# KiloHertzian/Open-Headstage

Hardware: AMD Instinct MI355X
Metric: Msamples/s stereo 48 kHz (4×512-tap HRIR conv + 10-band EQ); % HBM3E peak (higher is better)
Workload: dtype f32

## Files before the change

### open_headstage_amd/csrc/eq_quad_ring_body.hpp

```cpp
#pragma once
#include "kernels.h"
#include "eq_ring64_body.hpp"
#include "eq_quad_ring_asm.inc"
#include "eq_quad_ring_cl_asm.inc"
#include <type_traits>

namespace ohs {

constexpr int kQuadGroup = 16;
constexpr int kQuadK = EQ_QUAD_RING_K;
constexpr int kQp0003 = 0xC0, kQp0033 = 0xF0, kQp0012 = 0x90, kQp0101 = 0x44;

struct QuadRegs { float Z0, Z1, Zp, G, P; };
enum { kQuadLoopCluster, kQuadLoopLone, kQuadLoopFill };

template <int CTRL>
__device__ __forceinline__ float quad_dpp(float src)
{
    return __int_as_float(__builtin_amdgcn_update_dpp(0, __float_as_int(src), CTRL, 0xf, 0xf, true));
}

template <int LOOP = kQuadLoopCluster>
__device__ __forceinline__ void eq_quad_ring_wave(const float *in, float *out, long long stream_stride, long long ch_stride,
                                                  long long n, int n_chains, int nb, const EqPassTable &tab,
                                                  float *__restrict__ state, long long chain)
{
    constexpr int G = kQuadGroup, K = kQuadK;
    static_assert(K == 8, "the operand list below names x0 .. x7");
    static_assert(EQ_QUAD_RING_CL_HOLD == 1, "the clobber list below names one holding register, v20");
    if (chain >= n_chains) return;
    const int lane = threadIdx.x & 63, q = lane >> 2, role = lane & 3;
    const int n32 = (int)n;
    const bool band = q < nb, conv = q >= 12;
    const int j = band ? q : 0;
    const float C1 = role < 2 ? 1.0f : !band ? 0.0f : role == 2 ? tab.a2[j] : tab.a1[j];
    const float C2 = !band ? (role < 2 ? 0.0f : 1.0f) : role == 0 ? tab.b2[j] : role == 1 ? tab.b1[j] : role == 2 ? tab.b0[j] : 1.0f;
    const long long base = (chain >> 1) * stream_stride + (chain & 1) * ch_stride;
    const float *src0 = in + base;
    float *dst0 = out + base;
    float *state0 = state + chain * (kEqStateSlots * 2);
    const bool st_band = band && role >= 2;
    const unsigned state_off = (unsigned)(tab.slot[j] * 2 + (role == 2 ? 1 : 0)) * 4u;
    const float s_init = st_band ? ring2_ld(state0, state_off) : 0.0f;
    float s_save = s_init;
    const int t_in = 4 * q + 2;
    const int xs = (role == 0 ? 71 : role == 1 ? 69 : role == 2 ? 62 : 60) - 4 * q;
    const int ss = (role == 0 ? -1 : -3) - 4 * q;
    const bool st_lane = conv && (role == 0 || role == 3), inj_lane = conv && role >= 2;
    auto load_x = [&](int g) -> float {
        const int i = g * G + xs;
        return (conv && (unsigned)i < (unsigned)n32) ? ring2_ld(src0, (unsigned)i * 4u) : 0.0f;
    };
    QuadRegs r = {0.0f, 0.0f, 0.0f, 0.0f, 0.0f};
    float xcur = load_x(-1), xnext = load_x(0);

    const int g_hi = (n32 + 1) / G;
    const int iters = g_hi - 5 >= K ? (g_hi - 5) / K : 0;
    const int g1 = iters ? g_hi : -1, g0 = iters ? g_hi - iters * K : -1;
    float x2 = 0.0f, x3 = 0.0f, x4 = 0.0f, x5 = 0.0f, x6 = 0.0f, x7 = 0.0f;
    if (iters) {
        x2 = load_x(g0 + 2); x3 = load_x(g0 + 3); x4 = load_x(g0 + 4);
        x5 = load_x(g0 + 5); x6 = load_x(g0 + 6); x7 = load_x(g0 + 7);
    }

    enum { kPlain, kStore, kInjectB, kInjectA };
    auto group_cpp = [&](int g, auto with_state) {
        constexpr bool STATE = decltype(with_state)::value;
        const float xnext2 = load_x(g + 2);
        auto step = [&](auto kind, float &zc, const float zo, int s) {
            const int stp = g * G + s;
            zc = quad_dpp<kWaveRor1>(r.Zp) + r.G;
            r.Zp = quad_dpp<kQp0003>(zo) * C2;
            if constexpr (kind() == kStore) {
                const int yi = stp + ss;
                if (st_lane && (unsigned)yi < (unsigned)n32) ring2_st(dst0, (unsigned)yi * 4u, zc);
            } else if constexpr (kind() == kInjectB) {
                const float xb = quad_dpp<kQp0101>(xcur);
                r.Zp = inj_lane ? xb : r.Zp;
            } else if constexpr (kind() == kInjectA) {
                r.Zp = inj_lane ? xnext : r.Zp;
            }
            r.P = quad_dpp<kQp0033>(zc) * C1;
            r.G = quad_dpp<kQp0012>(zc) - r.P;
            if constexpr (STATE) {
                r.G = (st_band && stp == t_in) ? s_init : r.G;
                s_save = (st_band && stp == n32 + t_in) ? r.G : s_save;
            }
        };
        using Plain = std::integral_constant<int, kPlain>;
        auto plain_pairs = [&](int s0, int s1) {
#pragma unroll 1
            for (int s = s0; s < s1; s += 2) {
                step(Plain{}, r.Z1, r.Z0, s);
                step(Plain{}, r.Z0, r.Z1, s + 1);
            }
        };
        plain_pairs(1, 6);
        step(Plain{}, r.Z1, r.Z0, 7);
        step(std::integral_constant<int, kStore>{}, r.Z0, r.Z1, 8);
        step(std::integral_constant<int, kInjectB>{}, r.Z1, r.Z0, 9);
        step(Plain{}, r.Z0, r.Z1, 10);
        plain_pairs(11, 14);
        step(std::integral_constant<int, kStore>{}, r.Z1, r.Z0, 15);
        step(std::integral_constant<int, kInjectA>{}, r.Z0, r.Z1, 16);
        xcur = xnext;
        xnext = xnext2;
    };

    const int g_total = (n32 + 62 + G - 1) / G;
    int g = -1;
    const int head_end = iters ? g0 : g_total;
#pragma unroll 1
    for (; g < head_end && (g < 3 || !iters); ++g) group_cpp(g, std::true_type{});
#pragma unroll 1
    for (; g < head_end; ++g) group_cpp(g, std::false_type{});
    if (iters) {
        const unsigned bytes = (unsigned)n32 * 4u;
        const ring64_rsrc_t rin = ring64_rsrc(src0, bytes), rout = ring64_rsrc(dst0, bytes);
        unsigned voff_st = st_lane ? (unsigned)(G * (g0 - 1) + 8 + ss) * 4u : 0xFFFFF000u;
        unsigned voff_ld = conv ? (unsigned)(G * g0 + xs) * 4u : 0xFFFFF000u;
        const unsigned inc_ld = conv ? 4u * G * K : 0u, inc_st = st_lane ? 4u * G * K : 0u;
        unsigned cnt = 0u - (unsigned)__builtin_amdgcn_readfirstlane(iters);
#ifdef OHS_EXPERIMENTS
        if constexpr (LOOP == kQuadLoopFill) {
            unsigned fill = 0u;
            asm volatile(
                "s_nop 4\n"
                EQ_QUAD_RING_LOOP_FILL
                : [Z0] "+{v2}"(r.Z0), [Z1] "+{v3}"(r.Z1), [Zp] "+{v4}"(r.Zp), [Gr] "+{v5}"(r.G), [P] "+{v6}"(r.P),
                  [vs] "+{v0}"(voff_st), [vl] "+{v1}"(voff_ld), [x0] "+{v11}"(xcur), [x1] "+{v12}"(xnext), [x2] "+{v13}"(x2),
                  [x3] "+{v14}"(x3), [x4] "+{v15}"(x4), [x5] "+{v16}"(x5), [x6] "+{v17}"(x6), [x7] "+{v18}"(x7),
                  [F] "+{v19}"(fill), [cnt] "+s"(cnt)
                : [C1] "{v7}"(C1), [C2] "{v8}"(C2), [incl] "{v9}"(inc_ld), [incs] "{v10}"(inc_st), [rin] "s"(rin), [rout] "s"(rout)
                : "memory", "scc", "vcc");
        } else if constexpr (LOOP == kQuadLoopLone) {
            asm volatile(
                "s_nop 4\n"
                EQ_QUAD_RING_LOOP
                : [Z0] "+{v2}"(r.Z0), [Z1] "+{v3}"(r.Z1), [Zp] "+{v4}"(r.Zp), [Gr] "+{v5}"(r.G), [P] "+{v6}"(r.P),
                  [vs] "+{v0}"(voff_st), [vl] "+{v1}"(voff_ld), [x0] "+{v11}"(xcur), [x1] "+{v12}"(xnext), [x2] "+{v13}"(x2),
                  [x3] "+{v14}"(x3), [x4] "+{v15}"(x4), [x5] "+{v16}"(x5), [x6] "+{v17}"(x6), [x7] "+{v18}"(x7), [cnt] "+s"(cnt)
                : [C1] "{v7}"(C1), [C2] "{v8}"(C2), [incl] "{v9}"(inc_ld), [incs] "{v10}"(inc_st), [rin] "s"(rin), [rout] "s"(rout)
                : "memory", "scc", "vcc");
        } else
#endif
        asm volatile(
            "s_nop 4\n"
            EQ_QUAD_RING_CL_LOOP
            : [Z0] "+{v2}"(r.Z0), [Z1] "+{v3}"(r.Z1), [Zp] "+{v4}"(r.Zp), [Gr] "+{v5}"(r.G), [P] "+{v6}"(r.P),
              [vs] "+{v0}"(voff_st), [vl] "+{v1}"(voff_ld), [x0] "+{v11}"(xcur), [x1] "+{v12}"(xnext), [x2] "+{v13}"(x2),
              [x3] "+{v14}"(x3), [x4] "+{v15}"(x4), [x5] "+{v16}"(x5), [x6] "+{v17}"(x6), [x7] "+{v18}"(x7), [cnt] "+s"(cnt)
            : [C1] "{v7}"(C1), [C2] "{v8}"(C2), [incl] "{v9}"(inc_ld), [incs] "{v10}"(inc_st), [rin] "s"(rin), [rout] "s"(rout)
            : "memory", "scc", "vcc", "v20");
        g = g1;
#pragma unroll 1
        for (; g < g_total; ++g) group_cpp(g, std::true_type{});
    }
    if (st_band) ring2_st(state0, state_off, s_save);
}

}
```

Baseline: 27340.

## Rewrite quad-ring head/tail with buffer ops and 8-deep rotating prefetch

Restructures the C++ head and tail of the quad-ring EQ kernel. Loads and stores now go through raw buffer intrinsics with an out-of-range sentinel offset instead of branches. The head loop is unrolled into an 8-register rotating prefetch that mirrors the asm steady-state loop. Stores are deferred to a per-group port step, and the state injection and extraction are split so each part only runs where it is needed. The aim is to remove divergent branches and load latency stalls in the prologue and epilogue. The cost is more code, dummy stores at the start, and some risk in the index alignment logic.

```diff
diff --git a/open_headstage_amd/csrc/eq_quad_ring_body.hpp b/open_headstage_amd/csrc/eq_quad_ring_body.hpp
--- a/open_headstage_amd/csrc/eq_quad_ring_body.hpp
+++ b/open_headstage_amd/csrc/eq_quad_ring_body.hpp
@@ -9,6 +9,7 @@
 
 constexpr int kQuadGroup = 16;
 constexpr int kQuadK = EQ_QUAD_RING_K;
+constexpr unsigned kQuadNoSample = 0xFFFFF000u;
 constexpr int kQp0003 = 0xC0, kQp0033 = 0xF0, kQp0012 = 0x90, kQp0101 = 0x44;
 
 struct QuadRegs { float Z0, Z1, Zp, G, P; };
@@ -43,52 +44,60 @@
     const unsigned state_off = (unsigned)(tab.slot[j] * 2 + (role == 2 ? 1 : 0)) * 4u;
     const float s_init = st_band ? ring2_ld(state0, state_off) : 0.0f;
     float s_save = s_init;
-    const int t_in = 4 * q + 2;
+    const int t_in = st_band ? 4 * q + 2 : -0x40000000;
     const int xs = (role == 0 ? 71 : role == 1 ? 69 : role == 2 ? 62 : 60) - 4 * q;
     const int ss = (role == 0 ? -1 : -3) - 4 * q;
     const bool st_lane = conv && (role == 0 || role == 3), inj_lane = conv && role >= 2;
-    auto load_x = [&](int g) -> float {
-        const int i = g * G + xs;
-        return (conv && (unsigned)i < (unsigned)n32) ? ring2_ld(src0, (unsigned)i * 4u) : 0.0f;
+    const unsigned bytes = (unsigned)n32 * 4u;
+    const ring64_rsrc_t rin = ring64_rsrc(src0, bytes), rout = ring64_rsrc(dst0, bytes);
+    const __amdgpu_buffer_rsrc_t bin = __builtin_amdgcn_make_buffer_rsrc(const_cast<float *>(src0), 0, (int)bytes, 0x00020000);
+    const __amdgpu_buffer_rsrc_t bout = __builtin_amdgcn_make_buffer_rsrc(dst0, 0, (int)bytes, 0x00020000);
+    auto lane_const = [](int v) __attribute__((always_inline)) -> int {
+        asm volatile("" : "+v"(v));
+        return v;
+    };
+    auto load_x = [&](int g) __attribute__((always_inline)) -> float {
+        const int i = g * G + lane_const(xs);
+        const unsigned off = (conv && (unsigned)i < (unsigned)n32) ? (unsigned)i * 4u : kQuadNoSample;
+        return __uint_as_float(__builtin_amdgcn_raw_buffer_load_b32(bin, (int)off, 0, 0));
+    };
+    auto store_y = [&](int stp, float v) __attribute__((always_inline)) {
+        const int yi = stp + lane_const(ss);
+        const unsigned off = (st_lane && (unsigned)yi < (unsigned)n32) ? (unsigned)yi * 4u : kQuadNoSample;
+        __builtin_amdgcn_raw_buffer_store_b32(__float_as_uint(v), bout, (int)off, 0, 0);
+    };
+    auto store_none = [&]() __attribute__((always_inline)) {
+        __builtin_amdgcn_raw_buffer_store_b32(0u, bout, lane_const((int)kQuadNoSample), 0, 0);
     };
     QuadRegs r = {0.0f, 0.0f, 0.0f, 0.0f, 0.0f};
-    float xcur = load_x(-1), xnext = load_x(0);
 
     const int g_hi = (n32 + 1) / G;
     const int iters = g_hi - 5 >= K ? (g_hi - 5) / K : 0;
     const int g1 = iters ? g_hi : -1, g0 = iters ? g_hi - iters * K : -1;
-    float x2 = 0.0f, x3 = 0.0f, x4 = 0.0f, x5 = 0.0f, x6 = 0.0f, x7 = 0.0f;
-    if (iters) {
-        x2 = load_x(g0 + 2); x3 = load_x(g0 + 3); x4 = load_x(g0 + 4);
-        x5 = load_x(g0 + 5); x6 = load_x(g0 + 6); x7 = load_x(g0 + 7);
-    }
 
-    enum { kPlain, kStore, kInjectB, kInjectA };
-    auto group_cpp = [&](int g, auto with_state) {
-        constexpr bool STATE = decltype(with_state)::value;
-        const float xnext2 = load_x(g + 2);
-        auto step = [&](auto kind, float &zc, const float zo, int s) {
+    enum { kPlain, kHold, kInjectB, kInjectA };
+    enum { kStateIn = 1, kStateOut = 2 };
+    auto group_steps = [&](int g, const float xb, const float xa, float &h8, auto with_state) __attribute__((always_inline)) {
+        constexpr int STATE = decltype(with_state)::value;
+        auto step = [&](auto kind, float &zc, const float zo, int s) __attribute__((always_inline)) {
             const int stp = g * G + s;
             zc = quad_dpp<kWaveRor1>(r.Zp) + r.G;
             r.Zp = quad_dpp<kQp0003>(zo) * C2;
-            if constexpr (kind() == kStore) {
-                const int yi = stp + ss;
-                if (st_lane && (unsigned)yi < (unsigned)n32) ring2_st(dst0, (unsigned)yi * 4u, zc);
+            if constexpr (kind() == kHold) {
+                h8 = zc;
             } else if constexpr (kind() == kInjectB) {
-                const float xb = quad_dpp<kQp0101>(xcur);
-                r.Zp = inj_lane ? xb : r.Zp;
+                const float b = quad_dpp<kQp0101>(xb);
+                r.Zp = inj_lane ? b : r.Zp;
             } else if constexpr (kind() == kInjectA) {
-                r.Zp = inj_lane ? xnext : r.Zp;
+                r.Zp = inj_lane ? xa : r.Zp;
             }
             r.P = quad_dpp<kQp0033>(zc) * C1;
             r.G = quad_dpp<kQp0012>(zc) - r.P;
-            if constexpr (STATE) {
-                r.G = (st_band && stp == t_in) ? s_init : r.G;
-                s_save = (st_band && stp == n32 + t_in) ? r.G : s_save;
-            }
+            if constexpr ((STATE & kStateIn) != 0) r.G = stp == lane_const(t_in) ? s_init : r.G;
+            if constexpr ((STATE & kStateOut) != 0) s_save = stp - n32 == lane_const(t_in) ? r.G : s_save;
         };
         using Plain = std::integral_constant<int, kPlain>;
-        auto plain_pairs = [&](int s0, int s1) {
+        auto plain_pairs = [&](int s0, int s1) __attribute__((always_inline)) {
 #pragma unroll 1
             for (int s = s0; s < s1; s += 2) {
                 step(Plain{}, r.Z1, r.Z0, s);
@@ -97,28 +106,48 @@
         };
         plain_pairs(1, 6);
         step(Plain{}, r.Z1, r.Z0, 7);
-        step(std::integral_constant<int, kStore>{}, r.Z0, r.Z1, 8);
+        step(std::integral_constant<int, kHold>{}, r.Z0, r.Z1, 8);
         step(std::integral_constant<int, kInjectB>{}, r.Z1, r.Z0, 9);
         step(Plain{}, r.Z0, r.Z1, 10);
         plain_pairs(11, 14);
-        step(std::integral_constant<int, kStore>{}, r.Z1, r.Z0, 15);
+        step(Plain{}, r.Z1, r.Z0, 15);
         step(std::integral_constant<int, kInjectA>{}, r.Z0, r.Z1, 16);
-        xcur = xnext;
-        xnext = xnext2;
+    };
+    auto group_port = [&](int g, float &xb, const float h8, auto with_load) __attribute__((always_inline)) {
+        store_y(g * G + 8, h8);
+        store_y(g * G + 15, r.Z1);
+        if constexpr (decltype(with_load)::value) xb = load_x(g + K);
     };
 
     const int g_total = (n32 + 62 + G - 1) / G;
-    int g = -1;
     const int head_end = iters ? g0 : g_total;
+    int g = iters ? g0 - (g0 + K) / K * K : -1;
+    auto first_x = [&](int gx) __attribute__((always_inline)) -> float {
+        store_none();
+        store_none();
+        return load_x(gx);
+    };
+    float x0 = first_x(g), x1 = first_x(g + 1), x2 = first_x(g + 2), x3 = first_x(g + 3);
+    float x4 = first_x(g + 4), x5 = first_x(g + 5), x6 = first_x(g + 6), x7 = first_x(g + 7);
+    auto head_group = [&](float &xb, const float &xa) __attribute__((always_inline)) {
+        float h8 = 0.0f;
+        if (g < -1 || g >= head_end) {
+        } else if (iters) {
+            group_steps(g, xb, xa, h8, std::integral_constant<int, kStateIn>{});
+        } else {
+            group_steps(g, xb, xa, h8, std::integral_constant<int, kStateIn | kStateOut>{});
+        }
+        group_port(g, xb, h8, std::true_type{});
+        ++g;
+    };
 #pragma unroll 1
-    for (; g < head_end && (g < 3 || !iters); ++g) group_cpp(g, std::true_type{});
-#pragma unroll 1
-    for (; g < head_end; ++g) group_cpp(g, std::false_type{});
+    do {
+        head_group(x0, x1); head_group(x1, x2); head_group(x2, x3); head_group(x3, x4);
+        head_group(x4, x5); head_group(x5, x6); head_group(x6, x7); head_group(x7, x0);
+    } while (g < head_end);
     if (iters) {
-        const unsigned bytes = (unsigned)n32 * 4u;
-        const ring64_rsrc_t rin = ring64_rsrc(src0, bytes), rout = ring64_rsrc(dst0, bytes);
-        unsigned voff_st = st_lane ? (unsigned)(G * (g0 - 1) + 8 + ss) * 4u : 0xFFFFF000u;
-        unsigned voff_ld = conv ? (unsigned)(G * g0 + xs) * 4u : 0xFFFFF000u;
+        unsigned voff_st = st_lane ? (unsigned)(G * (g0 - 1) + 8 + ss) * 4u : kQuadNoSample;
+        unsigned voff_ld = conv ? (unsigned)(G * g0 + xs) * 4u : kQuadNoSample;
         const unsigned inc_ld = conv ? 4u * G * K : 0u, inc_st = st_lane ? 4u * G * K : 0u;
         unsigned cnt = 0u - (unsigned)__builtin_amdgcn_readfirstlane(iters);
 #ifdef OHS_EXPERIMENTS
@@ -128,7 +157,7 @@
                 "s_nop 4\n"
                 EQ_QUAD_RING_LOOP_FILL
                 : [Z0] "+{v2}"(r.Z0), [Z1] "+{v3}"(r.Z1), [Zp] "+{v4}"(r.Zp), [Gr] "+{v5}"(r.G), [P] "+{v6}"(r.P),
-                  [vs] "+{v0}"(voff_st), [vl] "+{v1}"(voff_ld), [x0] "+{v11}"(xcur), [x1] "+{v12}"(xnext), [x2] "+{v13}"(x2),
+                  [vs] "+{v0}"(voff_st), [vl] "+{v1}"(voff_ld), [x0] "+{v11}"(x0), [x1] "+{v12}"(x1), [x2] "+{v13}"(x2),
                   [x3] "+{v14}"(x3), [x4] "+{v15}"(x4), [x5] "+{v16}"(x5), [x6] "+{v17}"(x6), [x7] "+{v18}"(x7),
                   [F] "+{v19}"(fill), [cnt] "+s"(cnt)
                 : [C1] "{v7}"(C1), [C2] "{v8}"(C2), [incl] "{v9}"(inc_ld), [incs] "{v10}"(inc_st), [rin] "s"(rin), [rout] "s"(rout)
@@ -138,7 +167,7 @@
                 "s_nop 4\n"
                 EQ_QUAD_RING_LOOP
                 : [Z0] "+{v2}"(r.Z0), [Z1] "+{v3}"(r.Z1), [Zp] "+{v4}"(r.Zp), [Gr] "+{v5}"(r.G), [P] "+{v6}"(r.P),
-                  [vs] "+{v0}"(voff_st), [vl] "+{v1}"(voff_ld), [x0] "+{v11}"(xcur), [x1] "+{v12}"(xnext), [x2] "+{v13}"(x2),
+                  [vs] "+{v0}"(voff_st), [vl] "+{v1}"(voff_ld), [x0] "+{v11}"(x0), [x1] "+{v12}"(x1), [x2] "+{v13}"(x2),
                   [x3] "+{v14}"(x3), [x4] "+{v15}"(x4), [x5] "+{v16}"(x5), [x6] "+{v17}"(x6), [x7] "+{v18}"(x7), [cnt] "+s"(cnt)
                 : [C1] "{v7}"(C1), [C2] "{v8}"(C2), [incl] "{v9}"(inc_ld), [incs] "{v10}"(inc_st), [rin] "s"(rin), [rout] "s"(rout)
                 : "memory", "scc", "vcc");
@@ -148,13 +177,18 @@
             "s_nop 4\n"
             EQ_QUAD_RING_CL_LOOP
             : [Z0] "+{v2}"(r.Z0), [Z1] "+{v3}"(r.Z1), [Zp] "+{v4}"(r.Zp), [Gr] "+{v5}"(r.G), [P] "+{v6}"(r.P),
-              [vs] "+{v0}"(voff_st), [vl] "+{v1}"(voff_ld), [x0] "+{v11}"(xcur), [x1] "+{v12}"(xnext), [x2] "+{v13}"(x2),
+              [vs] "+{v0}"(voff_st), [vl] "+{v1}"(voff_ld), [x0] "+{v11}"(x0), [x1] "+{v12}"(x1), [x2] "+{v13}"(x2),
               [x3] "+{v14}"(x3), [x4] "+{v15}"(x4), [x5] "+{v16}"(x5), [x6] "+{v17}"(x6), [x7] "+{v18}"(x7), [cnt] "+s"(cnt)
             : [C1] "{v7}"(C1), [C2] "{v8}"(C2), [incl] "{v9}"(inc_ld), [incs] "{v10}"(inc_st), [rin] "s"(rin), [rout] "s"(rout)
             : "memory", "scc", "vcc", "v20");
-        g = g1;
+        float xt = x0;
 #pragma unroll 1
-        for (; g < g_total; ++g) group_cpp(g, std::true_type{});
+        for (g = g1; g < g_total; ++g) {
+            float h8;
+            group_steps(g, xt, 0.0f, h8, std::integral_constant<int, kStateOut>{});
+            group_port(g, xt, h8, std::false_type{});
+            xt = 0.0f;
+        }
     }
     if (st_band) ring2_st(state0, state_off, s_save);
 }
```

After: 27330 (median of 2 runs). Within noise of the previous version (-0.0%).
